# BetterBelle/eco-dqn

Measured on NVIDIA B200. Metric: env-steps/sec incl. MPNN Q-eval, higher is better.
Workload: dtype bf16x2-split/f32

## Files before the change

eco-dqn_b200/csrc/mpnn_tc.cu:

```cuda
#include <cuda_bf16.h>
#include <stdlib.h>

#include "eco_common.cuh"
#include "tc_prims.cuh"
#include "mpnn_pack.cuh"
#include "env_step_device.cuh"

namespace eco {
namespace {

using namespace tc;

constexpr int NPMAX = 208;
constexpr int PACK_NPMAX = 192;
constexpr int CHUNK = 64;
constexpr int SUBS = 2;
constexpr int THREADS = 256 * SUBS;
constexpr int GROUP_THREADS = 128 * SUBS;
constexpr int NWARPS = THREADS / 32;
constexpr int ISSUERS = 4;
constexpr int LAUNCH_THREADS = THREADS + 32 * ISSUERS;

constexpr uint32_t T_ACC0 = 0;
constexpr uint32_t T_ACC1 = 208;
constexpr uint32_t T_WM = 336;
constexpr uint32_t T_WU = 400;
constexpr uint32_t T_WEF = 464;
constexpr uint32_t T_S = 208;
constexpr uint32_t T_D = 312;

constexpr int SM_A = 0;
constexpr int SM_H = SM_A + NPMAX * NPMAX * 2;
constexpr int SM_E = SM_H + 128 * NPMAX * 2;
constexpr int SM_T = SM_E + 128 * NPMAX * 2;
constexpr int SM_ABS = SM_H;
constexpr int SM_XF = SM_T + 128 * CHUNK * 2;
constexpr int SM_DEG = SM_T + 2 * 128 * CHUNK * 2;
constexpr int SM_QP = SM_DEG + NPMAX * 4;
constexpr int MAXCHUNKS = (NPMAX + CHUNK - 1) / CHUNK;
constexpr int SM_PP = SM_QP + 4 * NPMAX * 4;
constexpr int SM_MISC = SM_PP + MAXCHUNKS * SUBS * 64 * 4;
constexpr int SM_TOTAL = SM_MISC + 64 + 16 * 4 + 16 * 4;
static_assert(NPMAX * NPMAX * 2 <= 2 * 128 * NPMAX * 2, "|A| must fit in the H+E region");
static_assert(7 * NPMAX * 4 <= 128 * CHUNK * 2, "xf must fit in a chunk buffer");
static_assert(SM_TOTAL + 256 <= 227 * 1024, "shared memory budget (dynamic + static)");

__global__ void mpnn_pack_kernel(const eco_mpnn_t w, uint32_t* __restrict__ out) {
    const int idx = blockIdx.x * blockDim.x + threadIdx.x;
    if (idx >= PK_WORDS) return;
    if (idx >= PK_WPT) {
        const int k = (idx - PK_WPT) >> 6, f = (idx - PK_WPT) & 63;
        out[idx] = __float_as_uint(w.w_pool[f * 64 + k]);
        return;
    }
    const float* src;
    int kw, rel, base;
    if (idx < PK_WM) { src = w.w_edge_feat; kw = 32; rel = idx; base = PK_WEF; }
    else if (idx < PK_WU) { const int l = (idx - PK_WM) / (128 * 64); src = w.w_msg[l]; kw = 64; rel = (idx - PK_WM) % (128 * 64); base = PK_WM + l * 128 * 64; }
    else { const int l = (idx - PK_WU) / (128 * 64); src = w.w_upd[l]; kw = 64; rel = (idx - PK_WU) % (128 * 64); base = PK_WU + l * 128 * 64; }
    const int r = rel / kw, c = rel % kw;
    const int f = 16 * (r >> 5) + (r & 15), s = (r >> 4) & 1;
    const float a = src[f * (2 * kw) + 2 * c], b = src[f * (2 * kw) + 2 * c + 1];
    uint32_t hi, lo;
    split2(a, b, hi, lo);
    out[base + packed_index(r, c, kw)] = s ? lo : hi;
}

struct Ctx {
    unsigned char* smem;
    uint32_t tmem;
    uint64_t* bar_all;
    uint64_t* bar_grp;
    uint64_t* bar_g2;
    uint64_t* bar_g3;
    uint32_t phase_all, phase_grp, phase_g2, phase_g3;
    int tid, warp, lane, q, grp, sub;
    int N, NP, NB;
};

__device__ __forceinline__ int group0_blocks(int nblocks) { return min((nblocks + 1) / 2, 2 * (CHUNK / 16)); }
__device__ __forceinline__ void workers_sync() { asm volatile("bar.sync 3, %0;" ::"n"(THREADS) : "memory"); }
__device__ __forceinline__ void cta_stage_sync() {
    fence_proxy_async();
    tc_fence_before();
    workers_sync();
}
__device__ __forceinline__ void wait_all(Ctx& c) {
    mbar_wait(c.bar_all, c.phase_all);
    c.phase_all ^= 1;
    tc_fence_after();
}
__device__ __forceinline__ void wait_grp(Ctx& c) {
    mbar_wait(c.bar_grp, c.phase_grp);
    c.phase_grp ^= 1;
    tc_fence_after();
}
__device__ __forceinline__ void wait_g2(Ctx& c) {
    mbar_wait(c.bar_g2, c.phase_g2);
    c.phase_g2 ^= 1;
    tc_fence_after();
}
__device__ __forceinline__ void wait_g3(Ctx& c) {
    mbar_wait(c.bar_g3, c.phase_g3);
    c.phase_g3 ^= 1;
    tc_fence_after();
}

template <int KW>
__device__ __forceinline__ void ldg_weights(const Ctx& c, const uint32_t* __restrict__ pk, uint4 (&buf)[KW / (8 * SUBS)]) {
    constexpr int CGP = KW / (16 * SUBS);
    const int part = c.grp * SUBS + c.sub;
    const uint4* src = reinterpret_cast<const uint4*>(pk) + ((c.q * (KW / 8) + part * CGP) * 2) * 32 + c.lane;
#pragma unroll
    for (int i = 0; i < 2 * CGP; ++i) buf[i] = __ldg(src + i * 32);
}
template <int KW>
__device__ __forceinline__ void sttm_weights(const Ctx& c, const uint4 (&buf)[KW / (8 * SUBS)], uint32_t tcol) {
    constexpr int CGP = KW / (16 * SUBS);
    const int part = c.grp * SUBS + c.sub;
#pragma unroll
    for (int i = 0; i < CGP; ++i) {
        const uint4 a = buf[2 * i], b = buf[2 * i + 1];
        const uint32_t v[8] = {a.x, a.y, a.z, a.w, b.x, b.y, b.z, b.w};
        tmem_st_32x32b_x8(tmem_addr(c.tmem, 32 * c.q, tcol + (part * CGP + i) * 8), v);
    }
}

template <class Fn>
__device__ __forceinline__ void epilogue(const Ctx& c, uint32_t acc, int col0, int width, Fn fn) {
    for (int blk = c.sub; blk < width / 16; blk += SUBS) {
        uint32_t vh[8], vl[8];
        tmem_ld_16x256b_x2(tmem_addr(c.tmem, 32 * c.q, acc + col0 + 16 * blk), vh);
        tmem_ld_16x256b_x2(tmem_addr(c.tmem, 32 * c.q + 16, acc + col0 + 16 * blk), vl);
        tmem_ld_wait();
        float v[8];
#pragma unroll
        for (int i = 0; i < 8; i += 2)
            add2(v[i], v[i + 1], __uint_as_float(vh[i]), __uint_as_float(vh[i + 1]), __uint_as_float(vl[i]), __uint_as_float(vl[i + 1]));
        fn(16 * blk, v);
    }
}

__device__ __forceinline__ void store_block(const Ctx& c, unsigned char* buf, int node0, const float (&v)[8]) {
    const int rowoff = 16 * (c.lane >> 2) + 4 * (c.lane & 3);
#pragma unroll
    for (int half = 0; half < 2; ++half) {
        const int cb = (node0 >> 3) + half;
#pragma unroll
        for (int fr = 0; fr < 2; ++fr) {
            uint32_t hi, lo;
            split2(v[4 * half + 2 * fr], v[4 * half + 2 * fr + 1], hi, lo);
            unsigned char* p = buf + ((cb * 16 + 4 * c.q + fr) * 128) + rowoff;
            *reinterpret_cast<uint32_t*>(p) = hi;
            *reinterpret_cast<uint32_t*>(p + 2 * 128) = lo;
        }
    }
}

__device__ __forceinline__ void issue_part(const Ctx& c, uint32_t acc_col, uint32_t tw, const unsigned char* x, int cb0,
                                           int width , bool accumulate) {
    const uint32_t idesc = instr_desc_bf16(128, width, false, true);
    const uint32_t idesc_lo = instr_desc_bf16(64, width, false, true);
    const uint64_t d = smem_desc(smem_u32(x) + cb0 * 2048,  128,  2048);
#pragma unroll
    for (int i = 0; i < 8; ++i)
        mma_ts(c.tmem + acc_col, c.tmem + tw + 8 * (i >> 1), d + (uint64_t)(16 * i), (i & 1) ? idesc_lo : idesc, accumulate || i > 0);
}

struct FusedEnv {
    eco_env_t env;
    int32_t* hist_a;
    double* hist_r;
    double* hist_s;
    int n_steps;
};

template <bool PACKED, bool TLINE, bool FUSED = false>
__global__ void __launch_bounds__(LAUNCH_THREADS, 1)
mpnn_tc_kernel(const eco_graphs_t g, const eco_mpnn_t w, const int B, const int32_t* __restrict__ graph_idx,
               const float* __restrict__ xn, const float* __restrict__ xg, const float norm_max,
               float* __restrict__ q_out, int32_t* __restrict__ act_out, unsigned long long* __restrict__ dbg,
               const int packK, const FusedEnv fe) {
    extern __shared__ __align__(128) unsigned char smem[];
    int dbg_n = 0;
#define TL(id)                                                                                           \
    do {                                                                                                 \
        if (TLINE && dbg != nullptr && blockIdx.x == 0 && (threadIdx.x & 31) == 0 && dbg_n < 1024)       \
            dbg[(threadIdx.x >> 5) * 1024 + dbg_n++] = ((unsigned long long)(id) << 48) | (clock64() & 0xFFFFFFFFFFFFull); \
    } while (0)
    __shared__ uint64_t bars[9];
    __shared__ uint64_t sig[2];
    __shared__ uint64_t sdbar[4];
    __shared__ uint64_t tail_sig, tail_done;
    __shared__ uint64_t gsig[2][2];
    __shared__ uint64_t bar_ops[2];
    __shared__ uint32_t tmem_base_s;
    Ctx c;
    c.smem = smem; c.phase_all = 0; c.phase_grp = 0; c.phase_g2 = 0; c.phase_g3 = 0;
    c.tid = threadIdx.x; c.lane = c.tid & 31;
    c.warp = __shfl_sync(0xffffffffu, c.tid >> 5, 0);
    c.q = c.warp & 3; c.sub = (c.warp >> 2) % SUBS;
    c.grp = c.warp < NWARPS ? c.warp / (4 * SUBS) : (c.warp == NWARPS + 2 ? 1 : 0);
    const bool linear_issuer = c.warp == NWARPS + 1 || c.warp == NWARPS + 2;
    c.bar_all = &bars[0]; c.bar_grp = &bars[1 + c.grp]; c.bar_g2 = &bars[5 + c.grp]; c.bar_g3 = &bars[7 + c.grp];
    const int K = PACKED ? packK : 1;
    const int NPs = g.NP, Ns = g.N;
    c.NP = K * NPs; c.NB = c.NP >> 3; c.N = PACKED ? c.NP : g.N;
    const int N = c.N, NP = c.NP, NB = c.NB;
    const int N8 = PACKED ? NP : ((N + 7) & ~7);
    const int npacks = (B + K - 1) / K;
    const int n_e = (int)blockIdx.x < npacks ? (npacks - (int)blockIdx.x + (int)gridDim.x - 1) / (int)gridDim.x : 0;
    const int n_items = n_e * (FUSED ? fe.n_steps : 1);
    auto item_ep = [&](int it) {
        if (!FUSED) return (int)blockIdx.x + it * (int)gridDim.x;
        const int nw = n_e >> 1, span = 2 * fe.n_steps;
        const int wi = min(it / span, nw - 1);
        const int members = wi == nw - 1 ? n_e - 2 * wi : 2;
        return (int)blockIdx.x + (2 * wi + (it - wi * span) % members) * (int)gridDim.x;
    };
    auto vertex_ok = [&](int n) { return PACKED ? (n % NPs) < Ns : n < N; };
    float* rdmaxv = reinterpret_cast<float*>(smem + SM_A + PACK_NPMAX * PACK_NPMAX * 2);
    float* pp_blk = rdmaxv + PACK_NPMAX;
    float* pooled_e = pp_blk + (PACK_NPMAX / 16) * 64;
    float* tef = pooled_e + (PACK_NPMAX / 16) * 64;

    float* xf = reinterpret_cast<float*>(smem + SM_XF);
    float* rdeg = reinterpret_cast<float*>(smem + SM_DEG);
    float* qpart = reinterpret_cast<float*>(smem + SM_QP);
    float* ppart = reinterpret_cast<float*>(smem + SM_PP);
    float* pooled = ppart;
    float* s_c0 = reinterpret_cast<float*>(smem + SM_MISC);
    float* red_val = s_c0 + 16;
    int* red_idx = reinterpret_cast<int*>(s_c0 + 32);
    unsigned char* sA = smem + SM_A;
    unsigned char* sAbs = smem + SM_ABS;
    unsigned char* sH = smem + SM_H;
    unsigned char* sE = smem + SM_E;
    unsigned char* sT = smem + SM_T + c.grp * (128 * CHUNK * 2);
    const uint32_t acc1 = T_ACC1 + 64 * c.grp;
    const uint32_t* pk = reinterpret_cast<const uint32_t*>(w.packed);

    if (c.warp == 0) tmem_alloc(&tmem_base_s, 512);
    if (c.tid == 0) {
        for (int i = 0; i < 9; ++i) mbar_init(&bars[i], 1);
        mbar_init(&bar_ops[0], 1); mbar_init(&bar_ops[1], 1);
        mbar_init(&sig[0], 1); mbar_init(&sig[1], 1);
        for (int i = 0; i < 4; ++i) mbar_init(&gsig[i >> 1][i & 1], 4 * SUBS);
        for (int i = 0; i < 4; ++i) mbar_init(&sdbar[i], NWARPS);
        mbar_init(&tail_sig, 1); mbar_init(&tail_done, 1);
        fence_mbar_init();
    }
    tc_fence_before();
    __syncthreads();
    tc_fence_after();
    c.tmem = tmem_base_s;
    if (c.warp < 4 && N8 < NP) {
        const uint32_t z[8] = {0, 0, 0, 0, 0, 0, 0, 0};
        tmem_st_32x32b_x8(tmem_addr(c.tmem, 32 * c.q, T_ACC0 + N8), z);
        tmem_st_wait();
        tc_fence_before();
    }
    const float dmax_set = norm_max > 0.f ? norm_max : *g.dmax;
    const int nsteps_A = NP >> 4;
    const int nblocks = NP >> 4;
    const int nb0 = group0_blocks(nblocks), nb1 = nblocks - nb0;
    const int nch0 = nb0 >= 2 ? 2 : nb0, nch1 = nb1 >= 2 ? 2 : nb1;
    const int nchunks = nch0 + nch1;
    const int chunk_split = nch0;
    const int cs = c.grp == 0 ? 0 : nch0;
    const int ncols0 = 16 * nb0;
    uint32_t phase_half = 0, phase_other = 0, phase_tail = 0;
    const int nmine = (c.warp < NWARPS || linear_issuer) ? (c.grp == 0 ? nch0 : nch1) : 0;
    const int nbm = c.grp == 0 ? nb0 : nb1;
    const int cA0 = c.grp == 0 ? 0 : ncols0, cAw = nmine > 1 ? 16 * ((nbm + 1) / 2) : 16 * nbm;
    const int cB0 = cA0 + cAw, cBw = 16 * nbm - cAw;
    const int cAm = min(cAw, N8 - cA0), cBm = min(cBw, N8 - cB0);
    auto signal_issuer = [&](int k) {
        fence_proxy_async();
        tc_fence_before();
        __syncwarp();
        if (c.lane == 0) mbar_arrive(&gsig[c.grp][k & 1]);
    };

    auto fetch_ops = [&](int which, int pack) {
        unsigned char* dst = which ? smem + SM_ABS : smem + SM_A;
        if (!PACKED) {
            const uint32_t ops_bytes = (uint32_t)NP * NP * 2;
            const uint16_t* src = g.tc_ops + ((size_t)graph_idx[pack] * 2 + which) * NP * NP;
            mbar_expect_tx(&bar_ops[which], ops_bytes);
            bulk_g2s(dst, src, ops_bytes, &bar_ops[which]);
        } else {
            const int kk = min(K, B - pack * K), NBs = NPs >> 3;
            mbar_expect_tx(&bar_ops[which], (uint32_t)kk * NPs * NPs * 2);
            for (int j = 0; j < kk; ++j) {
                const uint16_t* src = g.tc_ops + ((size_t)graph_idx[pack * K + j] * 2 + which) * NPs * NPs;
                for (int cb = 0; cb < NBs; ++cb)
                    bulk_g2s(dst + ((size_t)(j * NBs + cb) * NB + j * NBs) * 128, src + (size_t)cb * NBs * 64, NBs * 128,
                             &bar_ops[which]);
            }
        }
    };
    auto fetch_ops_warp = [&](int which, int pack) {
        unsigned char* dst = which ? smem + SM_ABS : smem + SM_A;
        const int kk = min(K, B - pack * K), NBs = NPs >> 3;
        if (c.lane == 0) mbar_expect_tx(&bar_ops[which], (uint32_t)kk * NPs * NPs * 2);
        __syncwarp();
        for (int idx = c.lane; idx < kk * NBs; idx += 32) {
            const int j = idx / NBs, cb = idx % NBs;
            const uint16_t* src = g.tc_ops + ((size_t)graph_idx[pack * K + j] * 2 + which) * NPs * NPs;
            bulk_g2s(dst + ((size_t)(j * NBs + cb) * NB + j * NBs) * 128, src + (size_t)cb * NBs * 64, NBs * 128, &bar_ops[which]);
        }
        __syncwarp();
    };
    auto zero_image = [&](unsigned char* dst) {
        for (int off = c.tid * 16; off < NP * NP * 2; off += THREADS * 16)
            *reinterpret_cast<uint4*>(dst + off) = make_uint4(0, 0, 0, 0);
        fence_proxy_async();
    };
    if (PACKED) {
        if (c.warp < NWARPS) { zero_image(smem + SM_A); zero_image(smem + SM_ABS); }
        __syncthreads();
    }
    if (c.tid == 0 && n_items > 0) { fetch_ops(0, blockIdx.x); fetch_ops(1, blockIdx.x); }

    const bool has_v = c.tid < NP;
    float xin0 = 0.f, xin1 = 0.f, xin2 = 0.f, degv = 1.f;
    float4 gl = make_float4(0.f, 0.f, 0.f, 0.f);
    int gmaxdeg = 1;
    auto load_inputs = [&](int e) {
        if (!PACKED) {
            const int ge = graph_idx[e];
            if (has_v) {
                xin0 = xn[((size_t)e * 3 + 0) * NP + c.tid];
                xin1 = xn[((size_t)e * 3 + 1) * NP + c.tid];
                xin2 = xn[((size_t)e * 3 + 2) * NP + c.tid];
                degv = g.deg[(size_t)ge * NP + c.tid];
            }
            gl = *reinterpret_cast<const float4*>(xg + (size_t)e * 4);
            gmaxdeg = g.gstat[(size_t)ge * 4];
        } else {
            const int be = e * K + c.tid / NPs, v = c.tid % NPs;
            xin0 = xin1 = xin2 = 0.f; degv = 1.f; gmaxdeg = 1;
            gl = make_float4(0.f, 0.f, 0.f, 0.f);
            if (has_v && be < B) {
                const int ge = graph_idx[be];
                xin0 = xn[((size_t)be * 3 + 0) * NPs + v];
                xin1 = xn[((size_t)be * 3 + 1) * NPs + v];
                xin2 = xn[((size_t)be * 3 + 2) * NPs + v];
                degv = g.deg[(size_t)ge * NPs + v];
                gl = *reinterpret_cast<const float4*>(xg + (size_t)be * 4);
                gmaxdeg = g.gstat[(size_t)ge * 4];
            }
        }
    };
    const float bread = __ldg(w.b_read);
    auto readout_warp_a = [&]() -> float {
        TL(60);
        float pa = 0.f, pb = 0.f;
        for (int k = 0; k < nchunks * SUBS; ++k) { pa += ppart[k * 64 + c.lane]; pb += ppart[k * 64 + 32 + c.lane]; }
        pooled[c.lane] = pa / (float)N;
        pooled[32 + c.lane] = pb / (float)N;
        __syncwarp();
        const float4* wt = reinterpret_cast<const float4*>(pk + PK_WPT) + c.lane;
        const int f4 = 4 * (c.lane & 15), kpar = c.lane >> 4;
        float4 acc = make_float4(0.f, 0.f, 0.f, 0.f);
#pragma unroll 1
        for (int k0 = 0; k0 < 64; k0 += 32) {
            float4 a[16];
#pragma unroll
            for (int j = 0; j < 16; ++j) a[j] = __ldg(wt + (k0 / 2 + j) * 32);
#pragma unroll
            for (int j = 0; j < 16; ++j) {
                const float pv = pooled[k0 + 2 * j + kpar];
                acc.x = fmaf(a[j].x, pv, acc.x); acc.y = fmaf(a[j].y, pv, acc.y);
                acc.z = fmaf(a[j].z, pv, acc.z); acc.w = fmaf(a[j].w, pv, acc.w);
            }
        }
        acc.x += __shfl_xor_sync(0xffffffffu, acc.x, 16); acc.y += __shfl_xor_sync(0xffffffffu, acc.y, 16);
        acc.z += __shfl_xor_sync(0xffffffffu, acc.z, 16); acc.w += __shfl_xor_sync(0xffffffffu, acc.w, 16);
        const float4 wr = __ldg(reinterpret_cast<const float4*>(w.w_read + f4));
        float t = kpar == 0 ? fmaf(wr.x, fmaxf(acc.x, 0.f), fmaf(wr.y, fmaxf(acc.y, 0.f),
                              fmaf(wr.z, fmaxf(acc.z, 0.f), wr.w * fmaxf(acc.w, 0.f)))) : 0.f;
#pragma unroll
        for (int o = 16; o > 0; o >>= 1) t += __shfl_xor_sync(0xffffffffu, t, o);
        TL(62);
        return bread + t;
    };
    auto readout_warp_b = [&](const int be, const float c0v) {
        TL(63);
        float bv = -INFINITY;
        int bi = 0x7fffffff;
        for (int i = c.lane; i < N; i += 32) {
            const float qv = c0v + ((qpart[i] + qpart[NPMAX + i]) + (qpart[2 * NPMAX + i] + qpart[3 * NPMAX + i]));
            if (q_out) q_out[(size_t)be * NP + i] = qv;
            if (qv > bv) { bv = qv; bi = i; }
        }
#pragma unroll
        for (int o = 16; o > 0; o >>= 1) {
            const float ov = __shfl_xor_sync(0xffffffffu, bv, o);
            const int oi = __shfl_xor_sync(0xffffffffu, bi, o);
            if (ov > bv || (ov == bv && oi < bi)) { bv = ov; bi = oi; }
        }
        if (c.lane == 0 && act_out) act_out[be] = bi;
        if (FUSED)
            env_step_group<32, false>(g, fe.env, be, c.lane, true, ECO_POLICY_ACTIONS, bi, nullptr, nullptr, fe.hist_a, fe.hist_r, fe.hist_s);
        TL(64);
    };
    constexpr int XF_DEG = 4, XF_GL = 5, XF_GMAX = 6;
    float* wsm_e = xf + 7 * NPMAX;
    float* wsm_i = wsm_e + 63 * 8;
    auto stage_inputs = [&](int e) {
        const int i = c.tid - GROUP_THREADS, per_row = NP >> 2;
        const int ge = graph_idx[e];
        if (i < 4 * per_row) {
            const int row = i / per_row, col = 4 * (i % per_row);
            const float* src = row < 3 ? xn + ((size_t)e * 3 + row) * NP + col : g.deg + (size_t)ge * NP + col;
            float* dst = xf + (row < 3 ? row : XF_DEG) * NPMAX + col;
            asm volatile("cp.async.cg.shared.global [%0], [%1], 16;" ::"r"(smem_u32(dst)), "l"(src) : "memory");
        } else if (i == 4 * per_row) {
            asm volatile("cp.async.cg.shared.global [%0], [%1], 16;" ::"r"(smem_u32(xf + XF_GL * NPMAX)), "l"(xg + (size_t)e * 4) : "memory");
        } else if (i == 4 * per_row + 1) {
            asm volatile("cp.async.ca.shared.global [%0], [%1], 4;" ::"r"(smem_u32(xf + XF_GMAX * NPMAX)), "l"(g.gstat + (size_t)ge * 4) : "memory");
        }
        if (i < (63 * 8) / 4)
            asm volatile("cp.async.ca.shared.global [%0], [%1], 16;" ::"r"(smem_u32(wsm_e + 4 * i)), "l"(w.w_edge + 4 * i) : "memory");
        if (i < (64 * 7) / 4)
            asm volatile("cp.async.ca.shared.global [%0], [%1], 16;" ::"r"(smem_u32(wsm_i + 4 * i)), "l"(w.w_init + 4 * i) : "memory");
        asm volatile("cp.async.commit_group;" ::: "memory");
    };
    auto readout_packed_warp = [&](const int be) {
        TL(60);
        const int bpe = NPs >> 4;
        for (int idx = c.lane; idx < K * 64; idx += 32) {
            const int e = idx >> 6, f = idx & 63;
            float t = 0.f;
            for (int j = 0; j < bpe; ++j) t += pp_blk[(e * bpe + j) * 64 + f];
            pooled_e[idx] = t / (float)Ns;
        }
        __syncwarp();
        TL(61);
        constexpr int KMAX = PACK_NPMAX / 16;
        float p0[KMAX], p1[KMAX];
#pragma unroll
        for (int e = 0; e < KMAX; ++e) { p0[e] = 0.f; p1[e] = 0.f; }
        const float* wt = reinterpret_cast<const float*>(pk + PK_WPT) + c.lane;
#pragma unroll 1
        for (int k0 = 0; k0 < 64; k0 += 16) {
            float wa[16], wb[16];
#pragma unroll
            for (int j = 0; j < 16; ++j) { wa[j] = __ldg(wt + (k0 + j) * 64); wb[j] = __ldg(wt + (k0 + j) * 64 + 32); }
#pragma unroll
            for (int j = 0; j < 16; ++j) {
#pragma unroll
                for (int e = 0; e < KMAX; ++e) {
                    if (e < K) {
                        const float pv = pooled_e[e * 64 + k0 + j];
                        p0[e] = fmaf(wa[j], pv, p0[e]);
                        p1[e] = fmaf(wb[j], pv, p1[e]);
                    }
                }
            }
        }
        TL(62);
        const float wr0 = __ldg(w.w_read + c.lane), wr1 = __ldg(w.w_read + 32 + c.lane);
        __syncwarp();
#pragma unroll
        for (int e = 0; e < KMAX; ++e) {
            if (e < K) {
                tef[e * 64 + c.lane] = wr0 * fmaxf(p0[e], 0.f);
                tef[e * 64 + 32 + c.lane] = wr1 * fmaxf(p1[e], 0.f);
            }
        }
        __syncwarp();
        if (c.lane < K) {
            float c0v = bread;
            for (int f = 0; f < 64; ++f) c0v += tef[c.lane * 64 + f];
            pooled_e[c.lane] = c0v;
        }
        __syncwarp();
        TL(63);
        for (int e = 0, i0 = 0; e < K; ++e, i0 += NPs) {
            const int ep = be * K + e;
            const float c0v = pooled_e[e];
            for (int v = c.lane; v < NPs; v += 32) {
                const int i = i0 + v;
                const float qv = c0v + ((qpart[i] + qpart[NPMAX + i]) + (qpart[2 * NPMAX + i] + qpart[3 * NPMAX + i]));
                const bool ok = v < Ns && ep < B;
                if (ok && q_out) q_out[(size_t)ep * NPs + v] = qv;
                qpart[i] = ok ? qv : -INFINITY;
            }
        }
        __syncwarp();
        TL(65);
        for (int e = 0; e < K; ++e) {
            const int ep = be * K + e;
            float bv = -INFINITY;
            int bi = 0x7fffffff;
            for (int v = c.lane; v < Ns; v += 32) {
                const float qv = qpart[e * NPs + v];
                if (qv > bv) { bv = qv; bi = v; }
            }
#pragma unroll
            for (int o = 16; o > 0; o >>= 1) {
                const float ov = __shfl_xor_sync(0xffffffffu, bv, o);
                const int oi = __shfl_xor_sync(0xffffffffu, bi, o);
                if (ov > bv || (ov == bv && oi < bi)) { bv = ov; bi = oi; }
            }
            if (c.lane == 0 && ep < B && act_out) act_out[ep] = bi;
        }
        TL(64);
    };
    if (c.warp == NWARPS) {

        uint32_t sp0 = 0, sp1 = 0, sp2 = 0, op = 0;
        for (int it = 0; it < n_items; ++it) {
            mbar_wait(&bar_ops[0], op);
            mbar_wait(&bar_ops[1], op); op ^= 1u;
            TL(51);
            for (int r = 0; 4 * r < nsteps_A; ++r) {
                mbar_wait(&sdbar[r], sp0);
                tc_fence_after();
                if (r == 0) TL(50);
                if (elect_one()) {
                    const uint32_t idesc = instr_desc_bf16(128, N8, false, false);
                    const uint64_t bd_abs = smem_desc(smem_u32(sAbs), NB * 128, 128);
                    const uint64_t bd_a = smem_desc(smem_u32(sA), NB * 128, 128);
                    const uint64_t kstep = (uint64_t)((2 * NB * 128) >> 4);
                    for (int ks = 4 * r; ks < min(4 * r + 4, nsteps_A); ++ks) {
                        mma_ts(c.tmem + T_ACC0, c.tmem + T_S + 8 * ks, bd_abs + ks * kstep, idesc, ks > 0);
                        mma_ts(c.tmem + T_ACC0, c.tmem + T_D + 8 * ks, bd_a + ks * kstep, idesc, true);
                    }
                    if (4 * r + 4 >= nsteps_A) mma_commit(c.bar_all);
                }
                __syncwarp();
            }
            sp0 ^= 1u;
            TL(52);
            for (int l = 0; l < 3; ++l) {
                mbar_wait(&sig[1], sp1); sp1 ^= 1u;
                tc_fence_after();
                TL(53);
                if (elect_one()) {
                    const uint64_t ad = smem_desc(smem_u32(sH), 2048, 128);
                    const uint64_t bstep = (uint64_t)((2 * NB * 128) >> 4);
                    for (int half = 0; half < 2; ++half) {
                        const int n0 = half ? ncols0 : 0, ncols = half ? N8 - ncols0 : min(ncols0, N8);
                        if (ncols == 0) break;
                        const uint32_t idesc = instr_desc_bf16(128, ncols, false, false);
                        const uint64_t bd = smem_desc(smem_u32(sA) + (n0 >> 3) * 128, NB * 128, 128);
                        for (int ks = 0; ks < nsteps_A; ++ks)
                            mma_ss(c.tmem + T_ACC0 + n0, ad + (uint64_t)ks * (4096 >> 4), bd + ks * bstep, idesc, ks > 0);
                        mma_commit(&bars[3 + half]);
                    }
                }
                __syncwarp();
                TL(54);
            }
            if (PACKED && it + 1 < n_items) {
                mbar_wait(&bars[N8 > ncols0 ? 4 : 3], (uint32_t)((3 * it + 2) & 1));
                fetch_ops_warp(0, item_ep(it + 1));
                mbar_wait(&sig[0], sp2); sp2 ^= 1u;
                fetch_ops_warp(1, item_ep(it + 1));
            }
        }
    }
    if (c.warp == NWARPS + 3) {
        uint32_t ph = 0;
        for (int it = 0; it < n_items - (PACKED ? 1 : 0); ++it) {
            mbar_wait(&tail_sig, ph);
            ph ^= 1u;
            if (PACKED) readout_packed_warp(item_ep(it));
            else readout_warp_b(item_ep(it), readout_warp_a());
            if (FUSED) __threadfence();
            __syncwarp();
            if (c.lane == 0) mbar_arrive(&tail_done);
        }
    }
    if (linear_issuer && nmine > 0) {
        uint32_t ph[2] = {0, 0};
        auto wait_sig = [&](int k) {
            mbar_wait(&gsig[c.grp][k & 1], ph[k & 1]);
            ph[k & 1] ^= 1u;
            tc_fence_after();
        };
        for (int it = 0; it < n_items; ++it) {
            wait_sig(0);
            if (elect_one()) { issue_part(c, T_ACC0 + cA0, T_WEF, sE, cA0 >> 3, cAm, false); mma_commit(c.bar_grp); }
            __syncwarp();
            if (nmine > 1) {
                wait_sig(1);
                if (elect_one()) { issue_part(c, acc1, T_WEF, sE, cB0 >> 3, cBm, false); mma_commit(c.bar_g2); }
                __syncwarp();
            }
            for (int l = 0; l < 3; ++l) {
                wait_sig(0);
                if (elect_one()) issue_part(c, acc1, T_WM + 32, sE, cA0 >> 3, cAm, false);
                __syncwarp();
                wait_sig(1);
                if (elect_one()) {
                    issue_part(c, acc1, T_WM, sT, 0, cAm, true);
                    mma_commit(c.bar_grp);
                    issue_part(c, T_ACC0 + cA0, T_WU, sH, cA0 >> 3, cAm, false);
                    mma_commit(c.bar_g2);
                }
                __syncwarp();
                if (nmine > 1) {
                    wait_sig(0);
                    if (elect_one()) {
                        issue_part(c, T_ACC0 + cB0, T_WU, sH, cB0 >> 3, cBm, false);
                        mma_commit(c.bar_g3);
                    }
                    __syncwarp();
                }
                wait_sig(1);
                if (elect_one()) {
                    issue_part(c, T_ACC0 + cA0, T_WU + 32, sH, cA0 >> 3, cAm, true);
                    mma_commit(c.bar_grp);
                    if (nmine > 1) {
                        issue_part(c, acc1, T_WM + 32, sE, cB0 >> 3, cBm, false);
                        issue_part(c, acc1, T_WM, sT, 0, cBm, true);
                        mma_commit(c.bar_g2);
                    }
                }
                __syncwarp();
                if (nmine > 1) {
                    wait_sig(0);
                    if (elect_one()) {
                        issue_part(c, T_ACC0 + cB0, T_WU + 32, sH, cB0 >> 3, cBm, true);
                        mma_commit(c.bar_grp);
                    }
                    __syncwarp();
                }
            }
        }
    }
    if (c.warp < NWARPS && n_items > 0) {
        {
            uint4 wef[32 / (8 * SUBS)];
            ldg_weights<32>(c, pk + PK_WEF, wef);
            sttm_weights<32>(c, wef, T_WEF);
            tmem_st_wait();
            tc_fence_before();
            workers_sync();
        }
        if (PACKED) load_inputs(blockIdx.x);
        else if (c.grp == 1) stage_inputs(blockIdx.x);
    }

    auto readout_packed_all = [&](const int be) {
        if (PACKED) {
            const int bpe = NPs >> 4;
            for (int idx = c.tid; idx < K * 64; idx += THREADS) {
                const int e = idx >> 6, f = idx & 63;
                float t = 0.f;
                for (int j = 0; j < bpe; ++j) t += pp_blk[(e * bpe + j) * 64 + f];
                pooled_e[idx] = t / (float)Ns;
            }
            workers_sync();
            for (int idx = c.tid; idx < K * 64; idx += THREADS) {
                const int e = idx >> 6, f = idx & 63;
                const float4* wp = reinterpret_cast<const float4*>(w.w_pool + f * 64);
                const float* pv = pooled_e + e * 64;
                float p = 0.f;
#pragma unroll 4
                for (int k4 = 0; k4 < 16; ++k4) {
                    const float4 wv = __ldg(wp + k4);
                    p = fmaf(wv.x, pv[4 * k4], p); p = fmaf(wv.y, pv[4 * k4 + 1], p);
                    p = fmaf(wv.z, pv[4 * k4 + 2], p); p = fmaf(wv.w, pv[4 * k4 + 3], p);
                }
                tef[idx] = __ldg(w.w_read + f) * fmaxf(p, 0.f);
            }
            workers_sync();
            if (c.tid < NP) {
                const int i = c.tid, e = i / NPs, v = i % NPs, ep = be * K + e;
                float c0v = bread;
                for (int f = 0; f < 64; ++f) c0v += tef[e * 64 + f];
                const float qv = c0v + ((qpart[i] + qpart[NPMAX + i]) + (qpart[2 * NPMAX + i] + qpart[3 * NPMAX + i]));
                const bool ok = v < Ns && ep < B;
                if (ok && q_out) q_out[(size_t)ep * NPs + v] = qv;
                qpart[i] = ok ? qv : -INFINITY;
            }
            workers_sync();
            for (int e = c.warp; e < K; e += NWARPS) {
                const int ep = be * K + e;
                float bv = -INFINITY;
                int bi = 0x7fffffff;
                for (int v = c.lane; v < Ns; v += 32) {
                    const float qv = qpart[e * NPs + v];
                    if (qv > bv) { bv = qv; bi = v; }
                }
#pragma unroll
                for (int o = 16; o > 0; o >>= 1) {
                    const float ov = __shfl_xor_sync(0xffffffffu, bv, o);
                    const int oi = __shfl_xor_sync(0xffffffffu, bi, o);
                    if (ov > bv || (ov == bv && oi < bi)) { bv = ov; bi = oi; }
                }
                if (c.lane == 0 && ep < B && act_out) act_out[ep] = bi;
            }
            workers_sync();
            return;
        }
    };
    int last_b = -1;

    for (int it = 0; it < n_items && c.warp < NWARPS; ++it) {
        const int b = item_ep(it);
        const bool has_next = it + 1 < n_items;
        const int b_next = has_next ? item_ep(it + 1) : 0;
        TL(1);
        if (!PACKED) {
            asm volatile("cp.async.wait_group 0;" ::: "memory");
            TL(70);
            workers_sync();
            TL(71);
            gl = *reinterpret_cast<const float4*>(xf + XF_GL * NPMAX);
            gmaxdeg = *reinterpret_cast<const int*>(xf + XF_GMAX * NPMAX);
            if (has_v) rdeg[c.tid] = __fdividef(1.f, xf[XF_DEG * NPMAX + c.tid]);
        }
        const float rdmax = __fdividef(1.f, norm_max < 0.f ? (float)max(gmaxdeg, 1) : dmax_set);

        const int fa = 16 * c.q + (c.lane >> 2), fb = fa + 8;
        float wxa[8], wxb[8], wia[7], wib[7];
        {
            const float* we = PACKED ? w.w_edge : wsm_e;
            const float* wi = PACKED ? w.w_init : wsm_i;
#pragma unroll
            for (int k = 0; k < 8; ++k) {
                wxa[k] = we[fa * 8 + k];
                wxb[k] = fb < 63 ? we[fb * 8 + k] : 0.f;
            }
#pragma unroll
            for (int k = 0; k < 7; ++k) { wia[k] = wi[fa * 7 + k]; wib[k] = wi[fb * 7 + k]; }
        }
        if (PACKED && has_v) {
            const int i = c.tid;
            const bool ok = vertex_ok(i);
            xf[0 * NPMAX + i] = ok ? xin0 : 0.f;
            xf[1 * NPMAX + i] = ok ? xin1 : 0.f;
            xf[2 * NPMAX + i] = ok ? xin2 : 0.f;
            rdeg[i] = __fdividef(1.f, degv);
            {
                xf[3 * NPMAX + i] = ok ? gl.x : 0.f;
                xf[4 * NPMAX + i] = ok ? gl.y : 0.f;
                xf[5 * NPMAX + i] = ok ? gl.z : 0.f;
                xf[6 * NPMAX + i] = ok ? gl.w : 0.f;
                rdmaxv[i] = 1.f / (norm_max < 0.f ? (float)max(gmaxdeg, 1) : dmax_set);
            }
        }
        float cxa = wxa[4] * gl.x, cxb = wxb[4] * gl.x, cia = wia[3] * gl.x, cib = wib[3] * gl.x;
        cxa = fmaf(wxa[5], gl.y, cxa); cxb = fmaf(wxb[5], gl.y, cxb); cia = fmaf(wia[4], gl.y, cia); cib = fmaf(wib[4], gl.y, cib);
        cxa = fmaf(wxa[6], gl.z, cxa); cxb = fmaf(wxb[6], gl.z, cxb); cia = fmaf(wia[5], gl.z, cia); cib = fmaf(wib[5], gl.z, cib);
        cxa = fmaf(wxa[7], gl.w, cxa); cxb = fmaf(wxb[7], gl.w, cxb); cia = fmaf(wia[6], gl.w, cia); cib = fmaf(wib[6], gl.w, cib);
        if (PACKED) { cxa = 0.f; cxb = 0.f; cia = 0.f; cib = 0.f; }
        constexpr int NOBS = PACKED ? 7 : 3;
        TL(2);
        if (PACKED) workers_sync();
        TL(3);
        {
            for (int r = 0; 4 * r < nsteps_A; ++r) {
                const int blk = 4 * r + c.grp * SUBS + c.sub;
                if (blk < nsteps_A) {
                uint32_t sh[4], sl[4], dh[4], dl[4];
#pragma unroll
                for (int half = 0; half < 2; ++half) {
                    const int n0 = 16 * blk + 8 * half + 2 * (c.lane & 3);
                    float pa0 = cxa, pa1 = cxa, pb0 = cxb, pb1 = cxb;
#pragma unroll
                    for (int k = 0; k < NOBS; ++k) {
                        const float2 x = *reinterpret_cast<const float2*>(xf + k * NPMAX + n0);
                        fma2(pa0, pa1, wxa[1 + k], wxa[1 + k], x.x, x.y, pa0, pa1);
                        fma2(pb0, pb1, wxb[1 + k], wxb[1 + k], x.x, x.y, pb0, pb1);
                    }
                    float rpa0, rpa1, rma0, rma1, rpb0, rpb1, rmb0, rmb1;
                    add2(rpa0, rpa1, pa0, pa1, wxa[0], wxa[0]); sub2(rma0, rma1, pa0, pa1, wxa[0], wxa[0]);
                    add2(rpb0, rpb1, pb0, pb1, wxb[0], wxb[0]); sub2(rmb0, rmb1, pb0, pb1, wxb[0], wxb[0]);
                    rpa0 = fmaxf(rpa0, 0.f); rpa1 = fmaxf(rpa1, 0.f); rma0 = fmaxf(rma0, 0.f); rma1 = fmaxf(rma1, 0.f);
                    rpb0 = fmaxf(rpb0, 0.f); rpb1 = fmaxf(rpb1, 0.f); rmb0 = fmaxf(rmb0, 0.f); rmb1 = fmaxf(rmb1, 0.f);
                    float sa0, sa1, sb0, sb1, da0, da1, db0, db1;
                    add2(sa0, sa1, rpa0, rpa1, rma0, rma1); add2(sb0, sb1, rpb0, rpb1, rmb0, rmb1);
                    sub2(da0, da1, rpa0, rpa1, rma0, rma1); sub2(db0, db1, rpb0, rpb1, rmb0, rmb1);
                    split2(sa0, sa1, sh[2 * half + 0], sl[2 * half + 0]);
                    split2(sb0, sb1, sh[2 * half + 1], sl[2 * half + 1]);
                    split2(da0, da1, dh[2 * half + 0], dl[2 * half + 0]);
                    split2(db0, db1, dh[2 * half + 1], dl[2 * half + 1]);
                }
                tmem_st_16x128b_x2(tmem_addr(c.tmem, 32 * c.q, T_S + 8 * blk), sh);
                tmem_st_16x128b_x2(tmem_addr(c.tmem, 32 * c.q + 16, T_S + 8 * blk), sl);
                tmem_st_16x128b_x2(tmem_addr(c.tmem, 32 * c.q, T_D + 8 * blk), dh);
                tmem_st_16x128b_x2(tmem_addr(c.tmem, 32 * c.q + 16, T_D + 8 * blk), dl);
                }
                tmem_st_wait();
                tc_fence_before();
                __syncwarp();
                if (c.lane == 0) mbar_arrive(&sdbar[r]);
            }
        }
        TL(4);
        {
            uint4 wm[64 / (8 * SUBS)], wu[64 / (8 * SUBS)];
            ldg_weights<64>(c, pk + PK_WM, wm);
            ldg_weights<64>(c, pk + PK_WU, wu);
            wait_all(c);
            TL(7);
            sttm_weights<64>(c, wm, T_WM);
            sttm_weights<64>(c, wu, T_WU);
        }

        {
            for (int k = 0; k < nmine; ++k) {
                const int c0 = k ? cB0 : cA0, width = k ? cBw : cAw;
                const bool has63 = c.q == 3 && (c.lane >> 2) == 7;
                epilogue(c, T_ACC0, c0, width, [&](int bc, float (&v)[8]) {
                    const int n0 = c0 + bc + 2 * (c.lane & 3);
                    const float2 r0 = *reinterpret_cast<const float2*>(rdeg + n0), r1 = *reinterpret_cast<const float2*>(rdeg + n0 + 8);
                    const float rd[4] = {r0.x, r0.y, r1.x, r1.y};
#pragma unroll
                    for (int i = 0; i < 8; i += 2) {
                        mul2(v[i], v[i + 1], v[i], v[i + 1], 0.5f, 0.5f);
                        mul2(v[i], v[i + 1], v[i], v[i + 1], rd[2 * (i >> 2)], rd[2 * (i >> 2) + 1]);
                    }
                    if (has63) {
#pragma unroll
                        for (int j = 0; j < 4; ++j) {
                            const int n = n0 + 8 * (j >> 1) + (j & 1);
                            v[2 + 4 * (j >> 1) + (j & 1)] = __fdividef(PACKED ? rdmaxv[n] : rdmax, rd[j]);
                        }
                    }
                    store_block(c, sE, c0 + bc, v);
                });
                signal_issuer(k);
                TL(10);
            }
        }
        {
            for (int blk = c.grp * SUBS + c.sub; blk < nsteps_A; blk += 2 * SUBS) {
                float v[8];
#pragma unroll
                for (int half = 0; half < 2; ++half) {
                    const int n0 = 16 * blk + 8 * half + 2 * (c.lane & 3);
                    float a0 = cia, a1 = cia, b0 = cib, b1 = cib;
#pragma unroll
                    for (int k = 0; k < NOBS; ++k) {
                        const float2 x = *reinterpret_cast<const float2*>(xf + k * NPMAX + n0);
                        fma2(a0, a1, wia[k], wia[k], x.x, x.y, a0, a1);
                        fma2(b0, b1, wib[k], wib[k], x.x, x.y, b0, b1);
                    }
                    v[4 * half + 0] = fmaxf(a0, 0.f); v[4 * half + 1] = fmaxf(a1, 0.f);
                    v[4 * half + 2] = fmaxf(b0, 0.f); v[4 * half + 3] = fmaxf(b1, 0.f);
                }
                store_block(c, sH, 16 * blk, v);
            }
        }
        tmem_st_wait();
        TL(8);
        auto epi_e = [&](uint32_t acc, int acc_col, int c0, int width) {
            epilogue(c, acc, acc_col, width, [&](int bc, float (&v)[8]) {
#pragma unroll
                for (int i = 0; i < 8; ++i) v[i] = fmaxf(v[i], 0.f);
                store_block(c, sE, c0 + bc, v);
            });
        };
        if (nmine > 0) {
            TL(15);
            wait_grp(c);
            TL(12);
            epi_e(T_ACC0, cA0, cA0, cAw);
            TL(13);
        }

        auto epi_agg = [&](int c0, int width, bool wait_b1) {
            bool waited = !wait_b1;
            epilogue(c, T_ACC0, c0, width, [&](int bc, float (&v)[8]) {
                const int n0 = c0 + bc + 2 * (c.lane & 3);
                const float2 r0 = *reinterpret_cast<const float2*>(rdeg + n0), r1 = *reinterpret_cast<const float2*>(rdeg + n0 + 8);
                const float rd[4] = {r0.x, r0.y, r1.x, r1.y};
#pragma unroll
                for (int i = 0; i < 8; i += 2) mul2(v[i], v[i + 1], v[i], v[i + 1], rd[2 * (i >> 2)], rd[2 * (i >> 2) + 1]);
                if (!waited) { wait_grp(c); waited = true; }
                store_block(c, sT, bc, v);
            });
            if (!waited) wait_grp(c);
        };
        auto epi_m = [&](int c0, int width) {
            epilogue(c, acc1, 0, width, [&](int bc, float (&v)[8]) {
#pragma unroll
                for (int i = 0; i < 8; ++i) v[i] = fmaxf(v[i], 0.f);
                store_block(c, sH, c0 + bc, v);
            });
        };
        for (int l = 0; l < 3; ++l) {
            TL(20);
            cta_stage_sync();
            TL(21);
            if (c.tid == 0) mbar_arrive(&sig[1]);
            if (l > 0) {
                uint4 wm[64 / (8 * SUBS)], wu[64 / (8 * SUBS)];
                ldg_weights<64>(c, pk + PK_WM + l * 128 * 64, wm);
                ldg_weights<64>(c, pk + PK_WU + l * 128 * 64, wu);
                sttm_weights<64>(c, wm, T_WM);
                sttm_weights<64>(c, wu, T_WU);
                tmem_st_wait();
                tc_fence_before();
                workers_sync();
            }
            if (l == 0 && nmine > 1) {
                wait_g2(c);
                epi_e(acc1, 0, cB0, cBw);
                TL(13);
            }
            if (nmine > 0) signal_issuer(0);
            TL(22);
            float wa = 0.f, wb = 0.f;
            if (l == 2) { wa = __ldg(w.w_read + 64 + fa); wb = __ldg(w.w_read + 64 + fa + 8); }
            if (l == 2 && last_b >= 0) {
                mbar_wait(&tail_done, phase_tail);
                phase_tail ^= 1u;
            }
            if (nmine > 0) {
                mbar_wait(&bars[3 + c.grp], phase_half);
                phase_half ^= 1u;
                tc_fence_after();
            }
            TL(23);
            if (!PACKED && l == 2 && c.tid == (chunk_split < nchunks ? THREADS / 2 : 0) && has_next) fetch_ops(0, b_next);
            auto epi_h = [&](int ci, int c0, int width) {
                if (l < 2) {
                    epilogue(c, T_ACC0, c0, width, [&](int bc, float (&v)[8]) {
#pragma unroll
                        for (int i = 0; i < 8; ++i) v[i] = fmaxf(v[i], 0.f);
                        store_block(c, sH, c0 + bc, v);
                    });
                    return;
                }
                float pool_a = 0.f, pool_b = 0.f;
                epilogue(c, T_ACC0, c0, width, [&](int bc, float (&v)[8]) {
                    float qv[4];
#pragma unroll
                    for (int j = 0; j < 4; ++j) {
                        const int ia = 4 * (j >> 1) + (j & 1), ib = ia + 2;
                        const int n = c0 + bc + 8 * (j >> 1) + 2 * (c.lane & 3) + (j & 1);
                        const float ha = fmaxf(v[ia], 0.f), hb = fmaxf(v[ib], 0.f);
                        if (vertex_ok(n)) { pool_a += ha; pool_b += hb; }
                        qv[j] = fmaf(wa, ha, wb * hb);
                    }
                    if (PACKED) {
                        pool_a += __shfl_xor_sync(0xffffffffu, pool_a, 1); pool_a += __shfl_xor_sync(0xffffffffu, pool_a, 2);
                        pool_b += __shfl_xor_sync(0xffffffffu, pool_b, 1); pool_b += __shfl_xor_sync(0xffffffffu, pool_b, 2);
                        if ((c.lane & 3) == 0) {
                            pp_blk[((c0 + bc) >> 4) * 64 + fa] = pool_a;
                            pp_blk[((c0 + bc) >> 4) * 64 + fa + 8] = pool_b;
                        }
                        pool_a = 0.f; pool_b = 0.f;
                    }
#pragma unroll
                    for (int j = 0; j < 4; ++j) {
                        qv[j] += __shfl_xor_sync(0xffffffffu, qv[j], 4);
                        qv[j] += __shfl_xor_sync(0xffffffffu, qv[j], 8);
                        qv[j] += __shfl_xor_sync(0xffffffffu, qv[j], 16);
                    }
                    if ((c.lane >> 2) == 0) {
#pragma unroll
                        for (int j = 0; j < 4; ++j)
                            qpart[c.q * NPMAX + c0 + bc + 8 * (j >> 1) + 2 * (c.lane & 3) + (j & 1)] = qv[j];
                    }
                });
                pool_a += __shfl_xor_sync(0xffffffffu, pool_a, 1); pool_a += __shfl_xor_sync(0xffffffffu, pool_a, 2);
                pool_b += __shfl_xor_sync(0xffffffffu, pool_b, 1); pool_b += __shfl_xor_sync(0xffffffffu, pool_b, 2);
                if (!PACKED && (c.lane & 3) == 0) {
                    ppart[(ci * SUBS + c.sub) * 64 + fa] = pool_a;
                    ppart[(ci * SUBS + c.sub) * 64 + fa + 8] = pool_b;
                }
            };
            if (nmine > 0) {
                epi_agg(cA0, cAw, false);
                signal_issuer(1);
                TL(30);
                if (nmine > 1) {
                    epi_agg(cB0, cBw, true);
                    signal_issuer(0);
                    TL(31);
                } else {
                    wait_grp(c);
                }
                wait_g2(c);
                if (c.grp == 0 && chunk_split < nchunks) {
                    mbar_wait(&bars[4], phase_other);
                    phase_other ^= 1u;
                }
                TL(33);
                epi_m(cA0, cAw);
                signal_issuer(1);
                TL(34);
                wait_grp(c);
                TL(37);
                epi_h(cs, cA0, cAw);
                TL(38);
                if (nmine > 1) {
                    wait_g2(c);
                    wait_g3(c);
                    if (!PACKED && l == 2 && c.grp == 1 && has_next) stage_inputs(b_next);
                    TL(33);
                    epi_m(cB0, cBw);
                    signal_issuer(0);
                    TL(35);
                    wait_grp(c);
                    TL(37);
                    epi_h(cs + 1, cB0, cBw);
                    TL(38);
                }
            }
        }
        TL(40);

        if (has_next) {
            if (PACKED) load_inputs(b_next);
            else if (c.grp == 1 && nmine < 2) stage_inputs(b_next);
        }
        workers_sync();
        if (PACKED && has_next) {
            TL(42);
            zero_image(smem + SM_ABS);
            workers_sync();
            TL(43);
        }
        if (c.tid == 0 && has_next) {
            if (PACKED) mbar_arrive(&sig[0]);
            else fetch_ops(1, b_next);
        }
        if (c.tid == 0 && (!PACKED || has_next)) mbar_arrive(&tail_sig);
        last_b = b;
        TL(41);
    }
    if (PACKED && c.warp < NWARPS && last_b >= 0) readout_packed_all(last_b);
#undef TL

    tc_fence_before();
    __syncthreads();
    if (c.warp == 0) tmem_dealloc(c.tmem, 512);
}

}

bool mpnn_tc_supported(const eco_graphs_t* g) { return g->N <= NPMAX && (g->reserved & ECO_GRAPHS_PM1) && g->tc_ops != nullptr; }
size_t mpnn_tc_scratch_bytes(int, int) { return (NWARPS + ISSUERS) * 1024 * 8 + 256; }
size_t mpnn_tc_packed_bytes() { return (size_t)PK_WORDS * 4; }

int launch_mpnn_pack(const eco_mpnn_t* w, void* packed, cudaStream_t st) {
    mpnn_pack_kernel<<<(PK_WORDS + 255) / 256, 256, 0, st>>>(*w, (uint32_t*)packed);
    ECO_LAUNCH_CHECK();
    return ECO_OK;
}

bool mpnn_tc_can_fuse(const eco_graphs_t* g, const eco_env_t* env) {
    const bool packed = PACK_NPMAX / g->NP >= 2 && env->B >= 2;
    return mpnn_tc_supported(g) && !packed && env->reserved == 0 && !(g->reserved & ECO_GRAPHS_MIN_CUT) && env->N == g->N &&
           env->B >= 2 * device_sm_count();
}

int launch_mpnn_tc(const eco_graphs_t* g, const eco_mpnn_t* w, int B, const int32_t* gidx, const float* xn,
                   const float* xg, float norm_max, float* q, int32_t* actions, void* scratch, cudaStream_t st) {
    return launch_mpnn_tc_fused(g, w, B, gidx, xn, xg, norm_max, q, actions, scratch, nullptr, 1, nullptr, nullptr, nullptr, st);
}

int launch_mpnn_tc_fused(const eco_graphs_t* g, const eco_mpnn_t* w, int B, const int32_t* gidx, const float* xn,
                         const float* xg, float norm_max, float* q, int32_t* actions, void* scratch, const eco_env_t* fused,
                         int n_steps, int32_t* ha, double* hr, double* hs, cudaStream_t st) {
    static unsigned long long attr_set = 0;
    const int n_sm = device_sm_count();
    if (first_use_on_device(&attr_set)) {
        ECO_CUDA((cudaFuncSetAttribute(mpnn_tc_kernel<false, false>, cudaFuncAttributeMaxDynamicSharedMemorySize, SM_TOTAL)));
        ECO_CUDA((cudaFuncSetAttribute(mpnn_tc_kernel<true, false>, cudaFuncAttributeMaxDynamicSharedMemorySize, SM_TOTAL)));
        ECO_CUDA((cudaFuncSetAttribute(mpnn_tc_kernel<false, true>, cudaFuncAttributeMaxDynamicSharedMemorySize, SM_TOTAL)));
        ECO_CUDA((cudaFuncSetAttribute(mpnn_tc_kernel<true, true>, cudaFuncAttributeMaxDynamicSharedMemorySize, SM_TOTAL)));
        ECO_CUDA((cudaFuncSetAttribute(mpnn_tc_kernel<false, false, true>, cudaFuncAttributeMaxDynamicSharedMemorySize, SM_TOTAL)));
    }
    const int packK = PACK_NPMAX / g->NP;
    const bool packed = packK >= 2 && B >= 2;
    if (fused && packed) { set_error("launch_mpnn_tc_fused: packed batches cannot be fused"); return ECO_ERR_INVALID; }
    const int units = packed ? (B + packK - 1) / packK : B;
    const int grid = units < n_sm ? units : n_sm;
    const int prof_kind = fused ? ECO_PROF_ROLLOUT : ECO_PROF_MPNN;
    prof_begin(prof_kind, st, fused ? n_steps : 1);
    static const bool timeline = getenv("ECO_TC_TIMELINE") != nullptr;
    if (timeline) ECO_CUDA(cudaMemsetAsync(scratch, 0, (NWARPS + ISSUERS) * 1024 * 8, st));
    unsigned long long* dbg = timeline ? (unsigned long long*)scratch : nullptr;
    FusedEnv fe{};
    fe.n_steps = 1;
    if (fused) {
        if (n_steps < 1 || B < 2 * grid) { set_error("launch_mpnn_tc_fused: needs n_steps >= 1 and two episodes per CTA"); return ECO_ERR_INVALID; }
        fe.env = *fused; fe.hist_a = ha; fe.hist_r = hr; fe.hist_s = hs; fe.n_steps = n_steps;
    }
    if (packed && dbg) mpnn_tc_kernel<true, true><<<grid, LAUNCH_THREADS, SM_TOTAL, st>>>(*g, *w, B, gidx, xn, xg, norm_max, q, actions, dbg, packK, fe);
    else if (packed) mpnn_tc_kernel<true, false><<<grid, LAUNCH_THREADS, SM_TOTAL, st>>>(*g, *w, B, gidx, xn, xg, norm_max, q, actions, nullptr, packK, fe);
    else if (dbg) mpnn_tc_kernel<false, true><<<grid, LAUNCH_THREADS, SM_TOTAL, st>>>(*g, *w, B, gidx, xn, xg, norm_max, q, actions, dbg, 1, fe);
    else if (fused) mpnn_tc_kernel<false, false, true><<<grid, LAUNCH_THREADS, SM_TOTAL, st>>>(*g, *w, B, gidx, xn, xg, norm_max, q, actions, nullptr, 1, fe);
    else mpnn_tc_kernel<false, false><<<grid, LAUNCH_THREADS, SM_TOTAL, st>>>(*g, *w, B, gidx, xn, xg, norm_max, q, actions, nullptr, 1, fe);
    prof_end(prof_kind, st);
    ECO_LAUNCH_CHECK();
    return ECO_OK;
}

}
```

Measured before the change: 7.778 million.

## Overlap init-embedding H computation with weight loads via early MMA commit barrier

Adds an mbarrier committed partway through the |A| MMA issue so the epilogue warps can start writing the init embedding H into the shared region it shares with |A|. That work now runs while the message and update weight global loads are in flight, instead of after they are staged into TMEM. The edge and init input weights are also staged into shared memory in a transposed float4 layout, so each thread reads its rows with a few vector loads rather than many scalar ones. Correctness depends on the commit point being late enough that the MMAs no longer read the overlapping smem region.

```diff
diff --git a/eco-dqn_b200/csrc/mpnn_tc.cu b/eco-dqn_b200/csrc/mpnn_tc.cu
--- a/eco-dqn_b200/csrc/mpnn_tc.cu
+++ b/eco-dqn_b200/csrc/mpnn_tc.cu
@@ -42,7 +42,7 @@
 constexpr int SM_MISC = SM_PP + MAXCHUNKS * SUBS * 64 * 4;
 constexpr int SM_TOTAL = SM_MISC + 64 + 16 * 4 + 16 * 4;
 static_assert(NPMAX * NPMAX * 2 <= 2 * 128 * NPMAX * 2, "|A| must fit in the H+E region");
-static_assert(7 * NPMAX * 4 <= 128 * CHUNK * 2, "xf must fit in a chunk buffer");
+static_assert((7 * NPMAX + 4 * 64 * 4) * 4 <= 128 * CHUNK * 2, "xf and the staged input weights must fit in a chunk buffer");
 static_assert(SM_TOTAL + 256 <= 227 * 1024, "shared memory budget (dynamic + static)");
 
 __global__ void mpnn_pack_kernel(const eco_mpnn_t w, uint32_t* __restrict__ out) {
@@ -191,6 +191,7 @@
     __shared__ uint64_t bars[9];
     __shared__ uint64_t sig[2];
     __shared__ uint64_t sdbar[4];
+    __shared__ uint64_t hbar;
     __shared__ uint64_t tail_sig, tail_done;
     __shared__ uint64_t gsig[2][2];
     __shared__ uint64_t bar_ops[2];
@@ -247,6 +248,7 @@
         mbar_init(&sig[0], 1); mbar_init(&sig[1], 1);
         for (int i = 0; i < 4; ++i) mbar_init(&gsig[i >> 1][i & 1], 4 * SUBS);
         for (int i = 0; i < 4; ++i) mbar_init(&sdbar[i], NWARPS);
+        mbar_init(&hbar, 1);
         mbar_init(&tail_sig, 1); mbar_init(&tail_done, 1);
         fence_mbar_init();
     }
@@ -269,7 +271,7 @@
     const int chunk_split = nch0;
     const int cs = c.grp == 0 ? 0 : nch0;
     const int ncols0 = 16 * nb0;
-    uint32_t phase_half = 0, phase_other = 0, phase_tail = 0;
+    uint32_t phase_half = 0, phase_other = 0, phase_tail = 0, phase_h = 0;
     const int nmine = (c.warp < NWARPS || linear_issuer) ? (c.grp == 0 ? nch0 : nch1) : 0;
     const int nbm = c.grp == 0 ? nb0 : nb1;
     const int cA0 = c.grp == 0 ? 0 : ncols0, cAw = nmine > 1 ? 16 * ((nbm + 1) / 2) : 16 * nbm;
@@ -408,7 +410,7 @@
     };
     constexpr int XF_DEG = 4, XF_GL = 5, XF_GMAX = 6;
     float* wsm_e = xf + 7 * NPMAX;
-    float* wsm_i = wsm_e + 63 * 8;
+    float* wsm_i = wsm_e + 2 * 64 * 4;
     auto stage_inputs = [&](int e) {
         const int i = c.tid - GROUP_THREADS, per_row = NP >> 2;
         const int ge = graph_idx[e];
@@ -423,9 +425,11 @@
             asm volatile("cp.async.ca.shared.global [%0], [%1], 4;" ::"r"(smem_u32(xf + XF_GMAX * NPMAX)), "l"(g.gstat + (size_t)ge * 4) : "memory");
         }
         if (i < (63 * 8) / 4)
-            asm volatile("cp.async.ca.shared.global [%0], [%1], 16;" ::"r"(smem_u32(wsm_e + 4 * i)), "l"(w.w_edge + 4 * i) : "memory");
-        if (i < (64 * 7) / 4)
-            asm volatile("cp.async.ca.shared.global [%0], [%1], 16;" ::"r"(smem_u32(wsm_i + 4 * i)), "l"(w.w_init + 4 * i) : "memory");
+            asm volatile("cp.async.ca.shared.global [%0], [%1], 16;" ::"r"(smem_u32(wsm_e + (i & 1) * 256 + 4 * (i >> 1))), "l"(w.w_edge + 4 * i) : "memory");
+        for (int j = i; j < 64 * 7; j += GROUP_THREADS) {
+            const int f = j / 7, k = j % 7;
+            asm volatile("cp.async.ca.shared.global [%0], [%1], 4;" ::"r"(smem_u32(wsm_i + (k >> 2) * 256 + 4 * f + (k & 3))), "l"(w.w_init + j) : "memory");
+        }
         asm volatile("cp.async.commit_group;" ::: "memory");
     };
     auto readout_packed_warp = [&](const int be) {
@@ -530,6 +534,7 @@
                         mma_ts(c.tmem + T_ACC0, c.tmem + T_S + 8 * ks, bd_abs + ks * kstep, idesc, ks > 0);
                         mma_ts(c.tmem + T_ACC0, c.tmem + T_D + 8 * ks, bd_a + ks * kstep, idesc, true);
                     }
+                    if (r == min(1, (nsteps_A - 1) >> 2)) mma_commit(&hbar);
                     if (4 * r + 4 >= nsteps_A) mma_commit(c.bar_all);
                 }
                 __syncwarp();
@@ -721,16 +726,25 @@
 
         const int fa = 16 * c.q + (c.lane >> 2), fb = fa + 8;
         float wxa[8], wxb[8], wia[7], wib[7];
-        {
-            const float* we = PACKED ? w.w_edge : wsm_e;
-            const float* wi = PACKED ? w.w_init : wsm_i;
+        if (PACKED) {
 #pragma unroll
             for (int k = 0; k < 8; ++k) {
-                wxa[k] = we[fa * 8 + k];
-                wxb[k] = fb < 63 ? we[fb * 8 + k] : 0.f;
-            }
-#pragma unroll
-            for (int k = 0; k < 7; ++k) { wia[k] = wi[fa * 7 + k]; wib[k] = wi[fb * 7 + k]; }
+                wxa[k] = w.w_edge[fa * 8 + k];
+                wxb[k] = fb < 63 ? w.w_edge[fb * 8 + k] : 0.f;
+            }
+#pragma unroll
+            for (int k = 0; k < 7; ++k) { wia[k] = w.w_init[fa * 7 + k]; wib[k] = w.w_init[fb * 7 + k]; }
+        } else {
+            const float4* we = reinterpret_cast<const float4*>(wsm_e);
+            const float4* wi = reinterpret_cast<const float4*>(wsm_i);
+            const float4 ea0 = we[fa], ea1 = we[64 + fa], eb0 = we[fb], eb1 = we[64 + fb];
+            const float4 ia0 = wi[fa], ia1 = wi[64 + fa], ib0 = wi[fb], ib1 = wi[64 + fb];
+            const bool r63 = fb == 63;
+            wxa[0] = ea0.x; wxa[1] = ea0.y; wxa[2] = ea0.z; wxa[3] = ea0.w; wxa[4] = ea1.x; wxa[5] = ea1.y; wxa[6] = ea1.z; wxa[7] = ea1.w;
+            wxb[0] = r63 ? 0.f : eb0.x; wxb[1] = r63 ? 0.f : eb0.y; wxb[2] = r63 ? 0.f : eb0.z; wxb[3] = r63 ? 0.f : eb0.w;
+            wxb[4] = r63 ? 0.f : eb1.x; wxb[5] = r63 ? 0.f : eb1.y; wxb[6] = r63 ? 0.f : eb1.z; wxb[7] = r63 ? 0.f : eb1.w;
+            wia[0] = ia0.x; wia[1] = ia0.y; wia[2] = ia0.z; wia[3] = ia0.w; wia[4] = ia1.x; wia[5] = ia1.y; wia[6] = ia1.z;
+            wib[0] = ib0.x; wib[1] = ib0.y; wib[2] = ib0.z; wib[3] = ib0.w; wib[4] = ib1.x; wib[5] = ib1.y; wib[6] = ib1.z;
         }
         if (PACKED && has_v) {
             const int i = c.tid;
@@ -796,15 +810,35 @@
             }
         }
         TL(4);
-        {
-            uint4 wm[64 / (8 * SUBS)], wu[64 / (8 * SUBS)];
-            ldg_weights<64>(c, pk + PK_WM, wm);
-            ldg_weights<64>(c, pk + PK_WU, wu);
-            wait_all(c);
-            TL(7);
-            sttm_weights<64>(c, wm, T_WM);
-            sttm_weights<64>(c, wu, T_WU);
-        }
+        uint4 wm[64 / (8 * SUBS)], wu[64 / (8 * SUBS)];
+        ldg_weights<64>(c, pk + PK_WM, wm);
+        ldg_weights<64>(c, pk + PK_WU, wu);
+        mbar_wait(&hbar, phase_h);
+        phase_h ^= 1u;
+        tc_fence_after();
+        TL(5);
+        for (int blk = c.grp * SUBS + c.sub; blk < nsteps_A; blk += 2 * SUBS) {
+            float v[8];
+#pragma unroll
+            for (int half = 0; half < 2; ++half) {
+                const int n0 = 16 * blk + 8 * half + 2 * (c.lane & 3);
+                float a0 = cia, a1 = cia, b0 = cib, b1 = cib;
+#pragma unroll
+                for (int k = 0; k < NOBS; ++k) {
+                    const float2 x = *reinterpret_cast<const float2*>(xf + k * NPMAX + n0);
+                    fma2(a0, a1, wia[k], wia[k], x.x, x.y, a0, a1);
+                    fma2(b0, b1, wib[k], wib[k], x.x, x.y, b0, b1);
+                }
+                v[4 * half + 0] = fmaxf(a0, 0.f); v[4 * half + 1] = fmaxf(a1, 0.f);
+                v[4 * half + 2] = fmaxf(b0, 0.f); v[4 * half + 3] = fmaxf(b1, 0.f);
+            }
+            store_block(c, sH, 16 * blk, v);
+        }
+        TL(8);
+        wait_all(c);
+        TL(7);
+        sttm_weights<64>(c, wm, T_WM);
+        sttm_weights<64>(c, wu, T_WU);
 
         {
             for (int k = 0; k < nmine; ++k) {
@@ -832,27 +866,7 @@
                 TL(10);
             }
         }
-        {
-            for (int blk = c.grp * SUBS + c.sub; blk < nsteps_A; blk += 2 * SUBS) {
-                float v[8];
-#pragma unroll
-                for (int half = 0; half < 2; ++half) {
-                    const int n0 = 16 * blk + 8 * half + 2 * (c.lane & 3);
-                    float a0 = cia, a1 = cia, b0 = cib, b1 = cib;
-#pragma unroll
-                    for (int k = 0; k < NOBS; ++k) {
-                        const float2 x = *reinterpret_cast<const float2*>(xf + k * NPMAX + n0);
-                        fma2(a0, a1, wia[k], wia[k], x.x, x.y, a0, a1);
-                        fma2(b0, b1, wib[k], wib[k], x.x, x.y, b0, b1);
-                    }
-                    v[4 * half + 0] = fmaxf(a0, 0.f); v[4 * half + 1] = fmaxf(a1, 0.f);
-                    v[4 * half + 2] = fmaxf(b0, 0.f); v[4 * half + 3] = fmaxf(b1, 0.f);
-                }
-                store_block(c, sH, 16 * blk, v);
-            }
-        }
         tmem_st_wait();
-        TL(8);
         auto epi_e = [&](uint32_t acc, int acc_col, int c0, int width) {
             epilogue(c, acc, acc_col, width, [&](int bc, float (&v)[8]) {
 #pragma unroll
```

Result: faster. 7.991 million, median of 6 (+2.7%).
